# zachtong/RAFT-DVC

Hardware: AMD Instinct MI355X
Metric: corr build+lookup voxel-queries/s (128^3 pair, 1/4 encoder) (higher is better)
Workload: dtype bf16; 1 GPU; corr build + 12 lookups, 32^3 x 128 fmaps (128^3 input, 1/4 encoder), L=4, r=4, materialised, bf16 build / fp32 lookup; global_batch=1, query_voxels=32768, levels=4, radius=4, parallelism=single GPU, step_replay=hip graph after the collective

## Files before the change

### include/dvccorr.h

```cpp
#ifndef DVCCORR_H
#define DVCCORR_H

#include <stddef.h>
#include <stdint.h>

#ifdef __cplusplus
extern "C" {
#endif

#define DVC_MAX_LEVELS 8
#define DVC_ABI_VERSION 3
#define DVC_CORR_GUARD_BYTES 256

typedef enum {
    DVC_OK = 0,
    DVC_ERR_INVALID = 1,
    DVC_ERR_UNSUPPORTED = 2,
    DVC_ERR_LAUNCH = 3,
    DVC_ERR_RUNTIME = 4
} dvc_status;

typedef enum { DVC_F32 = 0, DVC_BF16 = 1, DVC_F16 = 2 } dvc_dtype;

#define DVC_BRICKED 0x100

typedef enum { DVC_FIXED = 0, DVC_LEGACY = 1 } dvc_convention;

typedef struct {
    int32_t num_levels;
    int32_t channels;
    int32_t c_pad;
    int32_t H[DVC_MAX_LEVELS];
    int32_t W[DVC_MAX_LEVELS];
    int32_t D[DVC_MAX_LEVELS];
    int32_t Dp[DVC_MAX_LEVELS];
    int32_t zero_level[DVC_MAX_LEVELS];
    int64_t offset[DVC_MAX_LEVELS];
    int64_t level_elems[DVC_MAX_LEVELS];
    int64_t row_elems;
    int64_t row_stride;
} dvc_layout;

int dvc_layout_init(int H, int W, int D, int num_levels, int C, dvc_layout *out);

int dvc_bricked_levels(const dvc_layout *lay);

size_t dvc_pack_workspace_bytes(int B, int C, int H, int W, int D, int num_levels);

int dvc_pack_queries(const float *fmap1, void *packed, int B, int C, int64_t Nq, int dtype, void *stream);

int dvc_pack_targets(const float *fmap2, void *packed, float *workspace, int B, int C, int H, int W, int D,
                     int num_levels, int dtype, void *stream);

int dvc_pack_targets_gathered(const float *gathered, int world, void *packed, int B, int C, int H, int W, int D,
                              int num_levels, int dtype, void *stream);

int dvc_corr_build(const void *packed_q, const void *packed_t, void *corr, int B, int64_t Nq, int C, int H, int W,
                   int D, int num_levels, int in_dtype, int store_dtype, int64_t col_begin, int64_t col_end,
                   void *stream);

int dvc_corr_pool(void *corr, int B, int64_t Nq, int H, int W, int D, int num_levels, int src_level,
                  int store_dtype, void *stream);

int dvc_corr_lookup(const void *corr, const float *coords, float *out, int B, int64_t Nq, int H, int W, int D,
                    int num_levels, int radius, int convention, int store_dtype, void *stream);

size_t dvc_lookup_fused_workspace_bytes(int B, int64_t Nq, int num_levels, int radius);
int dvc_corr_lookup_fused(const void *packed_q, const void *packed_t, const float *coords, float *out,
                          void *workspace, int B, int64_t Nq, int C, int H, int W, int D, int num_levels,
                          int radius, int convention, int dtype, void *stream);

size_t dvc_corr_backward_workspace_bytes(int B, int64_t Nq, int C, int H, int W, int D, int num_levels, int radius);
size_t dvc_corr_backward_workspace_bytes_dtype(int B, int64_t Nq, int C, int H, int W, int D, int num_levels,
                                               int radius, int dtype);
int dvc_corr_backward(const void *packed_q, const void *packed_t, const float *coords, const float *grad_out,
                      float *grad_fmap1, float *grad_fmap2, void *workspace, int B, int64_t Nq, int C, int H, int W,
                      int D, int num_levels, int radius, int convention, int dtype, void *stream);
int dvc_corr_backward_mfma(int B, int64_t Nq, int C, int H, int W, int D, int num_levels, int radius, int convention,
// ... 136 lines not shown
```

### raft-dvc_amd/csrc/capi.hip

```cpp
#include <math.h>
#include <stdarg.h>
#include <stdio.h>
#include <stdlib.h>
#include <string.h>

#include "common.h"
#include "lookup_common.h"

#include <type_traits>

namespace dvc {
__global__ void k_pool_fmap(const float *, float *, long long, int, int, int, int, int, int);
template <typename T>
__global__ void k_pack_rows(const float *, T *, int, int, long long, long long, int, int, long long, long long);
template <typename T, int CG> __global__ void k_pack_pyramid(const float *, T *, PyrGeo);
template <typename T> __global__ void k_pack_queries(const float *, T *, int, int, long long);
template <int NCH, bool STORE_F32, int ABL>
__global__ void k_build_bf16(const bf16_t *, const bf16_t *, bf16_t *, long long, int, long long, long long, long long,
                             long long, int, float);
template <int NCH, typename E>
__global__ void k_build_bf16_2b(const E *, const E *, E *, long long, int, long long, long long,
                                long long, long long, int, float, int);
__global__ void k_build_f32(const float *, const float *, float *, long long, int, long long, long long, long long,
                            long long, int, float);
// ... 138 lines not shown
}

static int volume_check(const char *what, int B, int H, int W, int D, const char *indices = "indices") {
    if (B < 1 || H < 1 || W < 1 || D < 1) return fail(DVC_ERR_INVALID, "%s: B=%d volume (%d,%d,%d)", what, B, H, W, D);
    const long long vox = (long long)B * H * W * D;
    if (vox >= (1LL << 31)) return fail(DVC_ERR_UNSUPPORTED, "%s: %lld voxels exceed 32-bit %s", what, vox, indices);
    return DVC_OK;
}

static inline long long ceil_div(long long a, long long b) { return (a + b - 1) / b; }
static inline long long round_up(long long a, long long b) { return ceil_div(a, b) * b; }

static int fill_lookup_args(LookupArgs &A, const dvc_layout &lay, const void *corr, const float *coords, float *out,
                            int B, long long Nq, int radius, int convention) {
    A.corr = corr; A.coords = coords; A.out = out;
    A.Nq = Nq; A.q0 = 0; A.nq = Nq; A.row_stride = lay.row_stride; A.nqb = ceil_div(Nq, 64);
    A.B = B; A.Ltot = lay.num_levels; A.l0 = 0; A.nl = lay.num_levels;
    A.legacy = convention == DVC_LEGACY; A.r = radius;
    const int n = 2 * radius + 1;
    A.ach = n >= 3 ? 3 : n;
    A.nach = (int)ceil_div(n, A.ach);
    for (int l = 0; l < DVC_MAX_LEVELS; ++l) {
        A.H[l] = lay.H[l]; A.W[l] = lay.W[l]; A.D[l] = lay.D[l]; A.Dp[l] = lay.Dp[l];
        A.zero[l] = lay.zero_level[l]; A.off[l] = lay.offset[l];
        A.generic[l] = l < lay.num_levels && A.legacy && lay.W[l] != lay.D[l];
    }
    A.ablate = g_lookup_ablate;
    A.order = g_lookup_order;
    A.ldpol = g_lookup_ldpol;
    A.proj_w = nullptr; A.proj_b = nullptr; A.proj_out = nullptr;
    A.trace = (unsigned long long *)(((unsigned long long)(unsigned)g_trace_hi << 32) | (unsigned)g_trace_lo);
    A.split_levels = 0;
    A.brick = 0;
    return DVC_OK;
}


static int lookup_variant() {
    if (g_lookup_variant < 0) {
        const char *e = getenv("DVCCORR_LOOKUP_VARIANT");
        g_lookup_variant = e ? atoi(e) : 2;
    }
    return g_lookup_variant;
}

static bool tile_ok(const LookupArgs &A, size_t esz) {
    return A.r >= 1 && A.r <= 6 && (long long)64 * A.row_stride * (long long)esz < (1LL << 31) - 4096;
}

static constexpr long long kSplitTiles = 1024, kSplitRows = 512;
static Knob<int> g_split_ach{5};
static Knob<long long> g_split_tiles{kSplitTiles};
static Knob<int> g_lookup_waves{4};
static Knob<int> g_lookup_stpol{-1};

template <typename T, bool NT, int ACH>
static void launch_tile_r(const LookupArgs &A, dim3 blocks, unsigned threads, hipStream_t s) {
    switch (A.r) {
    case 1: k_lookup_tile<T, 1, NT, 0, false, ACH><<<blocks, threads, 0, s>>>(A); break;
    case 2: k_lookup_tile<T, 2, NT, 0, false, ACH><<<blocks, threads, 0, s>>>(A); break;
    case 3: k_lookup_tile<T, 3, NT, 0, false, ACH><<<blocks, threads, 0, s>>>(A); break;
    case 4: k_lookup_tile<T, 4, NT, 0, false, ACH><<<blocks, threads, 0, s>>>(A); break;
    case 5: k_lookup_tile<T, 5, NT, 0, false, ACH><<<blocks, threads, 0, s>>>(A); break;
    case 6: k_lookup_tile<T, 6, NT, 0, false, ACH><<<blocks, threads, 0, s>>>(A); break;
    default: break;
    }
}

template <typename T, bool NT>
static void launch_tile_nt(const LookupArgs &A0, hipStream_t s) {
    LookupArgs A = A0;
    const long long tiles = (long long)A.B * A.nqb;
    A.split_levels = tiles < g_split_tiles && A.nl > 1;
    const int n = 2 * A.r + 1;
    const int ach = g_split_ach;
    const bool split_rows = NT && A.split_levels && tiles * A.nl < kSplitRows && n > ach && ach > 0;
    const dim3 blocks((unsigned)tiles, A.split_levels ? (unsigned)A.nl : 1u,
                      split_rows ? (unsigned)((n + ach - 1) / ach) : 1u);
    const bool bal = NT && A.r == 4 && g_lookup_waves == 4 && (ach == 5 || !split_rows);
    const unsigned threads = 64u * (bal ? 4u : (unsigned)((2 * A.r + 3) / 3));
#if DVC_DIAG
    if constexpr (std::is_same<T, bf16_t>::value && NT) {
        if (A.r == 4 && A.ablate >= 1 && A.ablate <= 4) {
            const dim3 b1((unsigned)tiles, blocks.y);
            if (A.ablate == 4) k_lookup_tile<T, 4, NT, 4, false, 0><<<b1, 192, 0, s>>>(A);
            else if (A.ablate == 1) k_lookup_tile<T, 4, NT, 1, false, 0><<<b1, 192, 0, s>>>(A);
            else if (A.ablate == 2) k_lookup_tile<T, 4, NT, 2, false, 0><<<b1, 192, 0, s>>>(A);
            else k_lookup_tile<T, 4, NT, 3, false, 0><<<b1, 192, 0, s>>>(A);
            return;
        }
    }
#endif
    if constexpr (NT) {
        if (bal) {
#if DVC_DIAG
            if constexpr (std::is_same<T, bf16_t>::value) {
                if (A.trace) {
                    if (split_rows) k_lookup_tile<T, 4, true, 8, false, 5, 4><<<blocks, threads, 0, s>>>(A);
                    else k_lookup_tile<T, 4, true, 8, false, 0, 4><<<blocks, threads, 0, s>>>(A);
                    return;
                }
            }
#endif
            if (split_rows) {
                k_lookup_tile<T, 4, true, 0, false, 5, 4><<<blocks, threads, 0, s>>>(A);
                return;
            }
#if DVC_DIAG
            if constexpr (std::is_same<T, bf16_t>::value) {
                switch (g_lookup_stpol) {
// ... 95 lines not shown
#endif
    if (!strcmp(key, "lookup_variant")) {
        if (value < 0 || value > 2) return fail(DVC_ERR_INVALID, "set_tuning: lookup_variant %d", value);
        g_lookup_variant = value;
        return DVC_OK;
    }
    if (!strcmp(key, "lookup_stretch")) {
        if (value != 0 && value != 1) return fail(DVC_ERR_INVALID, "set_tuning: lookup_stretch %d (0 or 1)", value);
        g_lookup_stretch = value;
        return DVC_OK;
    }
    if (!strcmp(key, "lookup_nt")) {
        g_lookup_nt = value != 0;
        return DVC_OK;
    }
    if (!strcmp(key, "lookup_order")) {
        g_lookup_order = value != 0;
        return DVC_OK;
    }
    if (!strcmp(key, "lookup_ldpol")) {
        if (value < 0 || value > 3) return fail(DVC_ERR_INVALID, "set_tuning: lookup_ldpol %d", value);
        g_lookup_ldpol = value;
        return DVC_OK;
    }
    if (!strcmp(key, "lookup_waves")) {
        if (value != 0 && value != 4) return fail(DVC_ERR_INVALID, "set_tuning: lookup_waves %d (0 or 4)", value);
        g_lookup_waves = value;
        return DVC_OK;
    }
    if (!strcmp(key, "lookup_stpol")) {
        if (value != -1 && value != 0 && value != 16 && value != 17 && value != 18)
            return fail(DVC_ERR_INVALID, "set_tuning: lookup_stpol %d (-1, 0, 16, 17 or 18)", value);
        g_lookup_stpol = value;
        return DVC_OK;
    }
    if (!strcmp(key, "split_tiles")) {
        if (value < 0) return fail(DVC_ERR_INVALID, "set_tuning: split_tiles %d", value);
        g_split_tiles = value;
        return DVC_OK;
    }
    if (!strcmp(key, "split_ach")) {
        if (value != 0 && value != 2 && value != 3 && value != 5)
            return fail(DVC_ERR_INVALID, "set_tuning: split_ach %d (0, 2, 3 or 5)", value);
        g_split_ach = value;
        return DVC_OK;
    }
    if (!strcmp(key, "brick_min_dp")) {
        if (value != 16 && value != 32) return fail(DVC_ERR_INVALID, "set_tuning: brick_min_dp %d (16 or 32)", value);
        g_brick_min_dp = value;
        return DVC_OK;
    }
    if (!strcmp(key, "build_stpol")) {
        g_build_stpol = value != 0;
        return DVC_OK;
    }
    if (!strcmp(key, "pack_cg")) {
        if (value != 0 && value != 8 && value != 16 && value != 32) return fail(DVC_ERR_INVALID, "set_tuning: pack_cg %d", value);
        g_pack_cg = value;
        return DVC_OK;
    }
    if (!strcmp(key, "pack_variant")) {
        if (value < 0 || value > 1) return fail(DVC_ERR_INVALID, "set_tuning: pack_variant %d", value);
        g_pack_variant = value;
        return DVC_OK;
    }
    if (!strcmp(key, "build_f32_variant")) {
// ... 432 lines not shown
            return fail(DVC_ERR_UNSUPPORTED, "lookup: a DVC_BRICKED pyramid needs the tile kernel (radius 1..6, "
                                             "no legacy W != D bricked level, lookup_variant 2)");
    }
    const long long items = (long long)A.nl * A.nach * B * A.nqb;
    const unsigned blocks = (unsigned)ceil_div(items, 4);
    hipStream_t s = (hipStream_t)stream;
    if (store_dtype == DVC_BF16) launch_lookup<bf16_t>(A, blocks, s);
    else if (store_dtype == DVC_F16) launch_lookup<f16_t>(A, blocks, s);
    else launch_lookup<float>(A, blocks, s);
    if ((rc = check_launch("corr_lookup"))) return rc;
    if (radius >= 1 && radius <= 6) {
        for (int l = 0; l < lay.num_levels; ++l) {
            if (!A.generic[l] || A.zero[l]) continue;
            LookupArgs G = A;
            G.l0 = l; G.nl = 1;
            bool staged = false;
            if (store_dtype == DVC_BF16) staged = launch_stretch<bf16_t>(G, lay, l, s);
            else if (store_dtype == DVC_F16) staged = launch_stretch<f16_t>(G, lay, l, s);
            else staged = launch_stretch<float>(G, lay, l, s);
            if (staged) {
                if ((rc = check_launch("corr_lookup_stretch"))) return rc;
                continue;
            }
            const unsigned gb = (unsigned)ceil_div((long long)G.nach * B * G.nqb, 4);
            if (store_dtype == DVC_BF16) k_lookup_generic<bf16_t><<<gb, 256, 0, s>>>(G);
            else if (store_dtype == DVC_F16) k_lookup_generic<f16_t><<<gb, 256, 0, s>>>(G);
            else k_lookup_generic<float><<<gb, 256, 0, s>>>(G);
            if ((rc = check_launch("corr_lookup_generic"))) return rc;
        }
    }
    return DVC_OK;
}

size_t dvc_proj_packed_bytes(int num_levels, int radius) {
    if (num_levels < 1 || num_levels > DVC_MAX_LEVELS || radius < 1 || radius > DVC_PROJ_MAX_RADIUS) return 0;
    const int n = 2 * radius + 1;
    return (size_t)num_levels * n * ((n + 2) / 3) * DVC_PROJ_COUT * 32 * sizeof(bf16_t);
}

int dvc_proj_pack(const float *weight, void *packed, int cout, int num_levels, int radius, int convention,
                  void *stream) {
    if (!weight || !packed) return fail(DVC_ERR_INVALID, "proj_pack: null pointer");
    if (cout != DVC_PROJ_COUT) return fail(DVC_ERR_UNSUPPORTED, "proj_pack: %d output channels (convc1 has %d)", cout,
                                           DVC_PROJ_COUT);
    if (num_levels < 1 || num_levels > DVC_MAX_LEVELS)
        return fail(DVC_ERR_INVALID, "proj_pack: num_levels=%d outside [1, %d]", num_levels, DVC_MAX_LEVELS);
    if (radius < 1 || radius > DVC_PROJ_MAX_RADIUS)
        return fail(DVC_ERR_UNSUPPORTED, "proj_pack: radius %d outside [1, %d]", radius, DVC_PROJ_MAX_RADIUS);
    if (convention != DVC_FIXED && convention != DVC_LEGACY)
        return fail(DVC_ERR_INVALID, "proj_pack: bad convention %d", convention);
    const long long total = (long long)(dvc_proj_packed_bytes(num_levels, radius) / sizeof(bf16_t));
    k_proj_pack<<<(unsigned)ceil_div(total, 256), 256, 0, (hipStream_t)stream>>>(
        weight, (bf16_t *)packed, num_levels, radius, convention == DVC_LEGACY, total, 0);
    return check_launch("proj_pack");
}

int dvc_proj_pack_exact(const float *weight, void *packed, int cout, int num_levels, int radius, int convention,
                        void *stream) {
    if (!weight || !packed) return fail(DVC_ERR_INVALID, "proj_pack_exact: null pointer");
    if (cout != DVC_PROJ_COUT)
        return fail(DVC_ERR_UNSUPPORTED, "proj_pack_exact: %d output channels (convc1 has %d)", cout, DVC_PROJ_COUT);
    if (num_levels < 1 || num_levels > DVC_MAX_LEVELS)
        return fail(DVC_ERR_INVALID, "proj_pack_exact: num_levels=%d outside [1, %d]", num_levels, DVC_MAX_LEVELS);
    if (radius < 1 || radius > DVC_PROJ_MAX_RADIUS)
        return fail(DVC_ERR_UNSUPPORTED, "proj_pack_exact: radius %d outside [1, %d]", radius, DVC_PROJ_MAX_RADIUS);
    if (convention != DVC_FIXED && convention != DVC_LEGACY)
// ... 631 lines not shown
```

### raft-dvc_amd/csrc/common.h

```cpp
#pragma once

#include <hip/hip_runtime.h>
#include <stdint.h>

#include <algorithm>
#include <atomic>

#include "dvccorr.h"

#ifndef DVC_DIAG
#define DVC_DIAG 0
#endif
#ifndef DVC_PROJ_XLP
#define DVC_PROJ_XLP 0
#endif

typedef __bf16 bf16x2 __attribute__((ext_vector_type(2)));
typedef __bf16 bf16x8 __attribute__((ext_vector_type(8)));
typedef _Float16 f16x2 __attribute__((ext_vector_type(2)));
typedef _Float16 f16x8 __attribute__((ext_vector_type(8)));
typedef float f32x2 __attribute__((ext_vector_type(2)));
typedef float f32x4 __attribute__((ext_vector_type(4)));
typedef float f32x8 __attribute__((ext_vector_type(8)));
typedef float f32x16 __attribute__((ext_vector_type(16)));
// ... 31 lines not shown
}

__device__ __forceinline__ float bf16_bits_to_f32(unsigned int h) { return __uint_as_float(h << 16); }

__device__ __forceinline__ bf16_t f32_to_bf16(float f) { return __builtin_bit_cast(bf16_t, (__bf16)f); }

template <typename T> __device__ __forceinline__ unsigned pack2_16(float a, float b);
template <> __device__ __forceinline__ unsigned pack2_16<bf16_t>(float a, float b) {
    return (unsigned)f32_to_bf16(a) | ((unsigned)f32_to_bf16(b) << 16);
}
template <> __device__ __forceinline__ unsigned pack2_16<f16_t>(float a, float b) {
    return (unsigned)__builtin_bit_cast(unsigned short, (f16_t)a) |
           ((unsigned)__builtin_bit_cast(unsigned short, (f16_t)b) << 16);
}
template <typename T> __device__ __forceinline__ float bits16_to_f32(unsigned h);
template <> __device__ __forceinline__ float bits16_to_f32<bf16_t>(unsigned h) { return __uint_as_float(h << 16); }
template <> __device__ __forceinline__ float bits16_to_f32<f16_t>(unsigned h) {
    return (float)__builtin_bit_cast(f16_t, (unsigned short)(h & 0xffffu));
}

struct LookupArgs {
    const void *corr;
    const float *coords;
    float *out;
    long long Nq, q0, nq, nqb, row_stride;
    int B, Ltot, l0, nl, legacy, nach, ach, r;
    int H[DVC_MAX_LEVELS], W[DVC_MAX_LEVELS], D[DVC_MAX_LEVELS], Dp[DVC_MAX_LEVELS], zero[DVC_MAX_LEVELS];
    int generic[DVC_MAX_LEVELS];
    int ablate;
    int order;
    int ldpol;
    int split_levels;
    int brick;
    long long off[DVC_MAX_LEVELS];
    const void *proj_w;
    const float *proj_b;
    float *proj_out;
    unsigned long long *trace;
};

template <typename T> struct StoreT;
template <> struct StoreT<float> {
    static __device__ __forceinline__ float load(const float *p) { return *p; }
    static __device__ __forceinline__ void store(float *p, float v) { *p = v; }
};
template <> struct StoreT<bf16_t> {
    static __device__ __forceinline__ float load(const bf16_t *p) { return bf16_bits_to_f32(*p); }
    static __device__ __forceinline__ void store(bf16_t *p, float v) { *p = f32_to_bf16(v); }
};
template <> struct StoreT<f16_t> {
    static __device__ __forceinline__ float load(const f16_t *p) { return (float)*p; }
    static __device__ __forceinline__ void store(f16_t *p, float v) { *p = (f16_t)v; }
};

__device__ __forceinline__ float norm_coord(float x, float snm1) {
#pragma clang fp contract(off)
    float t = 2.0f * x;
    float u = t / snm1;
    return u - 1.0f;
}
__device__ __forceinline__ float unnorm_coord(float g, float sum1) {
#pragma clang fp contract(off)
    float t = g + 1.0f;
    float u = t / 2.0f;
    return u * sum1;
}
// ... 52 lines not shown
```

### raft-dvc_amd/csrc/lookup_common.h

```cpp
#pragma once

#include "common.h"

namespace dvc {

struct Item {
    int l, ac, b;
    long long qi;
};

__device__ __forceinline__ bool decode_item(const LookupArgs &A, Item &it) {
    const long long item = (long long)blockIdx.x * 4 + __builtin_amdgcn_readfirstlane((int)(threadIdx.x >> 6));
    const long long bq = (long long)A.B * A.nqb;
    const long long per_l = (long long)A.nach * bq;
    if (item >= per_l * A.nl) return false;
    const int li = (int)(item / per_l);
    long long rem = item - (long long)li * per_l;
    it.l = A.l0 + li;
    it.ac = (int)(rem / bq);
    rem -= (long long)it.ac * bq;
    it.b = (int)(rem / A.nqb);
    it.qi = (rem - (long long)it.b * A.nqb) * 64 + (threadIdx.x & 63);
    return true;
}
// ... 8 lines not shown

struct WinAxes {
    float ph, pu, pv;
    float kh, ku, kv;
    float hs, un, uu, vn, vu;
    bool dead;
};

__device__ __forceinline__ void window_axes(float py, float px, float pz, int Hl, int Wl, int Dl, int legacy,
                                            WinAxes &ax) {
    ax.ph = py;
    ax.pu = legacy ? pz : px;
    ax.pv = legacy ? px : pz;
    ax.dead = !(fabsf(ax.ph) < 1e6f) || !(fabsf(ax.pu) < 1e6f) || !(fabsf(ax.pv) < 1e6f);
    if (ax.dead) { ax.ph = -1e5f; ax.pu = -1e5f; ax.pv = -1e5f; }
    ax.hs = (float)(Hl - 1);
    ax.un = legacy ? (float)(Dl - 1) : (float)(Wl - 1);
    ax.uu = (float)(Wl - 1);
    ax.vn = legacy ? (float)(Wl - 1) : (float)(Dl - 1);
    ax.vu = (float)(Dl - 1);
    ax.kh = floorf(ax.ph);
    ax.ku = floorf(ax.pu);
    ax.kv = floorf(ax.pv);
}

__device__ __forceinline__ void axis_weights(float p, float kp, int d, float sn, float su, float &w0, float &w1) {
#pragma clang fp contract(off)
    const float x = roundtrip(p + (float)d, sn, su);
    const float k = kp + (float)d;
    w1 = x - k;
    w0 = (k + 1.0f) - x;
}

constexpr int kStretchSE = 3;
struct StretchGeo {
    int WX, DX, RB, LS, NYB, WXF;
    long long boxe;
};

}
```

### raft-dvc_amd/csrc/lookup_tile.h

```cpp
#pragma once

#include "common.h"
#include "lookup_common.h"

#include <type_traits>

namespace dvc {

#ifndef DVC_TILE_CB16
#define DVC_TILE_CB16 16
#endif
#ifndef DVC_TILE_PD16
#define DVC_TILE_PD16 2
#endif
template <typename T, int R, int NWV = 0> struct TileCfg {
    static constexpr int n = 2 * R + 1;
    static constexpr int NW = 2 * R + 2;
    static constexpr int ES = (int)sizeof(T);
    static constexpr int CB = ES == 4 ? 8 : (R <= 4 ? DVC_TILE_CB16 : 16);
    static constexpr int CE = CB / ES;
    static constexpr int ZWMAX = (NW + CE - 1 + CE - 1) / CE * CE;
    static constexpr int NWAVES = NWV > 0 ? NWV : (n + 2) / 3;
    static constexpr int COLS = NWV > 0 ? (n + NWV - 1) / NWV : 3;
    static constexpr int THREADS = 64 * NWAVES;
// ... 43 lines not shown
}

template <int NW>
__device__ __forceinline__ void lds_run(const unsigned char *base, int addr, const f16_t *, float (&v)[NW]) {
    constexpr int K = NW / 2;
    const unsigned *p = reinterpret_cast<const unsigned *>(base + (addr & ~3));
    unsigned d[K + 1];
#pragma unroll
    for (int i = 0; i <= K; ++i) d[i] = p[i];
    const unsigned sh = (unsigned)(addr & 2);
#pragma unroll
    for (int i = 0; i < K; ++i) {
        const unsigned w = __builtin_amdgcn_alignbyte(d[i + 1], d[i], sh);
        v[2 * i] = bits16_to_f32<f16_t>(w);
        v[2 * i + 1] = bits16_to_f32<f16_t>(w >> 16);
    }
}

template <int NW>
__device__ __forceinline__ void lds_run(const unsigned char *base, int addr, const float *, float (&v)[NW]) {
    const float *p = reinterpret_cast<const float *>(base + addr);
#pragma unroll
    for (int i = 0; i < NW; ++i) v[i] = p[i];
}

template <int n> struct ZRun {
    f32x2 p[n / 2];
    float t;
};

struct ProjCfg {
    static constexpr int COUT = 96, OT = COUT / 16, KW = 32;
};

#ifndef DVC_PROJ_ABL
#define DVC_PROJ_ABL 0
#endif
template <typename T, int R, bool NT, int ABL, int PROJ, int ACH, int NWV = 0, int SPOL = -1, bool XLP = false>
__global__ __launch_bounds__(64 * (TileCfg<T, R, NWV>::NWAVES + (PROJ ? 1 : 0)), PROJ == 2 ? 1 : 2) void k_lookup_tile(
    LookupArgs A) {
    using C = TileCfg<T, R, NWV>;
    static_assert(!PROJ || NWV == 0, "the convc1 weight packing assumes the 3-column waves");
    constexpr bool BAL = NWV > 0;
    constexpr int FLO = BAL ? C::n / C::NWAVES : 0, REM = BAL ? C::n % C::NWAVES : 0;
    constexpr int n = C::n, NW = C::NW, ES = C::ES, CE = C::CE, NP = n / 2;
    constexpr long long n3 = (long long)n * n * n;
    constexpr int NU_LAST = n - C::COLS * (C::NWAVES - 1);
    constexpr int XROW = C::NWAVES * ProjCfg::KW * 2 + 16;
    static_assert(!PROJ || C::COLS * n <= ProjCfg::KW, "PROJ: one wave's row values must fit a 32-k slice");
    __shared__ __attribute__((aligned(16))) unsigned char smem[C::LDS];
    __shared__ int tab[5][64];
    __shared__ __attribute__((aligned(16))) unsigned char xs[PROJ ? PROJ * 64 * XROW : 16];
    static_assert(PROJ != 2 || std::is_same<T, float>::value, "the split convc1 is the fp32 pyramid's");

    const int tid = threadIdx.x;
    const int lane = tid & 63;
    const int wave = __builtin_amdgcn_readfirstlane(tid >> 6);
    const int b = blockIdx.x / (int)A.nqb;
    const long long qb = blockIdx.x - (long long)b * A.nqb;
    const long long qt = qb * 64;
    const int nvalid = (int)min(64LL, A.nq - qt);
    const long long q = A.q0 + qt + lane;
    const bool active = lane < nvalid;
    const long long Nq = A.Nq;
    const bool rev = A.order && !A.split_levels && (blockIdx.x & 1);

    if constexpr (PROJ) {
        if (wave == C::NWAVES) {
            constexpr int OT = ProjCfg::OT, NWP = C::NWAVES;
            const int m16 = lane & 15, h4 = lane >> 4;
            f32x4 acc[OT][4];
#pragma unroll
            for (int ot = 0; ot < OT; ++ot)
#pragma unroll
                for (int j = 0; j < 4; ++j) acc[ot][j] = f32x4{0.f, 0.f, 0.f, 0.f};
            const f16x8 *wp = reinterpret_cast<const f16x8 *>(A.proj_w) + lane;
            const long long wlo = PROJ == 2 ? (long long)A.Ltot * n * NWP * OT * 64 : 0;
            const bool xlp_c = XLP && !A.split_levels;
            bool started_c = false;
            for (int li = 0; li < A.nl; ++li) {
                const int l = A.l0 + (rev ? A.nl - 1 - li : li);
                if (A.zero[l] || A.generic[l]) continue;
                if (!(xlp_c && started_c)) {
// ... 74 lines not shown
                for (int i = 0; i < 4; ++i) {
                    const int o = 16 * ot + 4 * h4 + i;
                    const float bo = A.proj_b[o];
#pragma unroll
                    for (int j = 0; j < 4; ++j) {
                        const int qq = 16 * j + m16;
                        const float v = acc[ot][j][i] + bo;
                        if (qq < nvalid) ob[(long long)o * Nq + qq] = v < 0.f ? 0.f : v;
                    }
                }
            return;
        }
    }

    const long long wg = ((long long)blockIdx.z * gridDim.y + blockIdx.y) * gridDim.x + blockIdx.x;
    int trace_level = 1;
    int trace_li = 0;
    auto stamp = [&](int k) {
        if constexpr ((ABL & 16) != 0) {
            if (tid == 0 && k < 16)
                __builtin_amdgcn_raw_buffer_store_b64(
                    __builtin_bit_cast(u32x2, (unsigned long long)__builtin_amdgcn_s_memrealtime()),
                    __builtin_amdgcn_make_buffer_rsrc(A.trace, (short)0, 0x7fffffff, 0x00020000),
                    (int)((wg * 64 + (k == 15 ? 3 : trace_li) * 16 + k) * 8), 0, 0);
        } else if constexpr ((ABL & 8) != 0) {
            if (tid == 0 && (trace_level || k == 15) && k < 16)
                __builtin_amdgcn_raw_buffer_store_b64(
                    __builtin_bit_cast(u32x2, (unsigned long long)__builtin_amdgcn_s_memrealtime()),
                    __builtin_amdgcn_make_buffer_rsrc(A.trace, (short)0, 0x7fffffff, 0x00020000),
                    (int)((wg * 16 + k) * 8), 0, 0);
        }
    };
    stamp(0);
    float cy = 0.f, cx = 0.f, cz = 0.f;
    if (active) load_coords(A.coords, b, Nq, q, cy, cx, cz);
    for (int i = tid * 16; i < C::LDS; i += C::THREADS * 16) *reinterpret_cast<u32x4 *>(smem + i) = u32x4{0, 0, 0, 0};

    const T *tile_rows = reinterpret_cast<const T *>(A.corr) + ((long long)b * Nq + A.q0 + qt) * A.row_stride;
    const unsigned long long trp = (unsigned long long)tile_rows;
    const unsigned trlo = __builtin_amdgcn_readfirstlane((unsigned)trp);
    const unsigned trhi = __builtin_amdgcn_readfirstlane((unsigned)(trp >> 32));
    const int nrec = __builtin_amdgcn_readfirstlane((int)((long long)nvalid * A.row_stride * ES));
    const __amdgpu_buffer_rsrc_t rs_in = __builtin_amdgcn_make_buffer_rsrc(
        (void *)(((unsigned long long)trhi << 32) | trlo), (short)0, nrec, 0x00020000);
    const int q4 = active ? (int)(q * 4) : 0x7ffffff0;
    const int chstep_u = A.legacy ? 1 : n;
    const int chstep_v = A.legacy ? n : 1;
    const int u0 = BAL ? wave * FLO + min(wave, REM) : wave * C::COLS;

    auto out_rsrc = [&](float *obase, int a, int u) {
        return __builtin_amdgcn_make_buffer_rsrc(obase + ((long long)a * n * n + (long long)u * chstep_u) * Nq,
                                                 (short)0, (int)(n * n * Nq * 4), 0x00020000);
    };
    auto store = [&](__amdgpu_buffer_rsrc_t rs, int v, float val) {
        if constexpr ((ABL & 1) != 0) asm volatile("" ::"v"(val));
        else __builtin_amdgcn_raw_buffer_store_b32(__float_as_uint(val), rs, q4, (int)(v * chstep_v * Nq * 4),
                                                   SPOL >= 0 ? SPOL : (NT ? 2 : 0));
    };

    static_assert(!PROJ || ACH == 0, "the convc1 consumer accumulates every row of the tile");
    using Chunk = typename std::conditional<C::CB == 16, u32x4, u32x2>::type;
    constexpr int PD = PROJ ? 2 : C::PD;
    const bool xlp = XLP && ACH == 0 && PD == 2 && !A.split_levels;
    Chunk st_x[PD][C::MAXCH];
    int voff[C::MAXCH];
    unsigned pk[C::MAXCH];
// ... 298 lines not shown
                u32x4 *dst = reinterpret_cast<u32x4 *>(xs + lane * XROW + wave * (ProjCfg::KW * 2));
#pragma unroll
                for (int j = 0; j < ProjCfg::KW / 8; ++j)
                    dst[j] = u32x4{xw[4 * j], xw[4 * j + 1], xw[4 * j + 2], xw[4 * j + 3]};
                if constexpr (PROJ == 2) {
                    u32x4 *dl = reinterpret_cast<u32x4 *>(xs + 64 * XROW + lane * XROW + wave * (ProjCfg::KW * 2));
#pragma unroll
                    for (int j = 0; j < ProjCfg::KW / 8; ++j)
                        dl[j] = u32x4{xwl[4 * j], xwl[4 * j + 1], xwl[4 * j + 2], xwl[4 * j + 3]};
                }
            }
            if (ia + 2 < NPL) {
                write_plane(ia & 1, a + 2, st[(ia + 2) % PD]);
                if (PD > 2 && ia + 2 + PD < NPL) load_plane(a + 2 + PD, g.plane_bytes, st[(ia + 2) % PD]);
            }
            if constexpr (XLP && PD == 2 && NA >= 3) {
                if (ia == NA - 3 && lnx >= 0 && wave == 0) {
                    const LevelGeo gn = geo(lnx);
                    WinAxes axn;
                    int ihn, iun, ivn, csn, zan;
                    window(lnx, gn, axn, ihn, iun, ivn, csn, zan);
                    write_tab(gn, ihn, csn, zan, ivn, iun);
                }
                if (ia == NA - 1 && lnx >= 0) {
                    write_plane(0, 0, st[0]);
                    load_plane(2, gx.plane_bytes, st[0]);
                }
            }
            __syncthreads();
            stamp(6 + ia);
        }
    };

    const int li0 = A.split_levels ? (int)blockIdx.y : 0;
    const int li1 = A.split_levels ? li0 + 1 : A.nl;
    constexpr int NCH_A = ACH > 0 ? (n + ACH - 1) / ACH : 1;
    constexpr int NA_FULL = ACH > 0 ? ACH : n;
    constexpr int NA_TAIL = ACH > 0 ? n - ACH * (NCH_A - 1) : n;
    const int a0 = ACH > 0 ? (int)blockIdx.z * ACH : 0;
    auto rows = [&](int l, auto nu_c, bool pre, int lnx) {
        if (NA_TAIL == NA_FULL || a0 + NA_FULL <= n) level(l, nu_c, std::integral_constant<int, NA_FULL>{}, a0, pre, lnx);
        else level(l, nu_c, std::integral_constant<int, NA_TAIL>{}, a0, pre, lnx);
    };
    auto walk_level = [&](int li) { return A.l0 + (rev ? A.nl - 1 - li : li); };
    auto runs = [&](int l) { return !A.zero[l] && !A.generic[l]; };
    bool started = false;
    for (int li = li0; li < li1; ++li) {
        const int l = walk_level(li);
        if (A.generic[l] && !A.zero[l]) continue;
        int lnx = -1;
        if (xlp && runs(l))
            for (int lj = li + 1; lj < li1 && lnx < 0; ++lj)
                if (runs(walk_level(lj))) lnx = walk_level(lj);
        const bool pre = xlp && started && runs(l);
        if constexpr (BAL) {
            if (REM > 0 && wave < REM) rows(l, std::integral_constant<int, FLO + 1>{}, pre, lnx);
            else rows(l, std::integral_constant<int, FLO>{}, pre, lnx);
        } else if (NU_LAST == C::COLS || wave < C::NWAVES - 1) {
            rows(l, std::integral_constant<int, C::COLS>{}, pre, lnx);
        } else {
            rows(l, std::integral_constant<int, NU_LAST>{}, pre, lnx);
        }
        started |= runs(l);
        trace_level = 0;
        ++trace_li;
    }
    stamp(15);
// ... 4 lines not shown
```

### raft-dvc_amd/dvccorr/_lib.py

```python
from __future__ import annotations

import ctypes
import os

_HERE = os.path.dirname(os.path.abspath(__file__))
LIB_PATH = os.environ.get("DVCCORR_LIB") or os.path.join(_HERE, "libdvccorr.so")

DVC_OK, DVC_ERR_INVALID, DVC_ERR_UNSUPPORTED, DVC_ERR_LAUNCH, DVC_ERR_RUNTIME = range(5)
DVC_F32, DVC_BF16, DVC_F16 = 0, 1, 2
DVC_BRICKED = 0x100
DVC_FIXED, DVC_LEGACY = 0, 1
MAX_LEVELS = 8

EXPORTED = (
    "dvc_layout_init", "dvc_pack_workspace_bytes", "dvc_pack_queries", "dvc_pack_targets", "dvc_pack_targets_gathered",
    "dvc_corr_build",
    "dvc_corr_pool", "dvc_corr_lookup", "dvc_lookup_fused_workspace_bytes", "dvc_corr_lookup_fused",
    "dvc_sample3d", "dvc_set_tuning", "dvc_last_error", "dvc_version", "dvc_abi_version",
    "dvc_corr_backward_workspace_bytes", "dvc_corr_backward_workspace_bytes_dtype", "dvc_corr_backward",
    "dvc_proj_packed_bytes", "dvc_proj_pack", "dvc_proj_pack_exact",
    "dvc_corr_lookup_proj", "dvc_lookup_fused_proj_workspace_bytes", "dvc_corr_lookup_fused_proj",
    "dvc_coords_grid", "dvc_upflow", "dvc_flow_step", "dvc_bricked_levels", "dvc_corr_backward_mfma", "dvc_corr_backward_gout64",
    "dvc_gru_packed_bytes", "dvc_gru_pack", "dvc_sep_gru_pass",
    "dvc_conv3_packed_bytes", "dvc_conv3_pack", "dvc_conv3",
    "dvc_conv7_flow_packed_bytes", "dvc_conv7_flow_pack", "dvc_conv7_flow",
    "dvc_conv3_pack_dgrad", "dvc_conv3_grad_prep", "dvc_conv3_wgrad_workspace_bytes", "dvc_conv3_wgrad",
    "dvc_sep_gru_pass_save", "dvc_gru_dgrad_packed_bytes", "dvc_gru_pack_dgrad", "dvc_gru_grad_prep",
    "dvc_sep_gru_dgrad", "dvc_gru_wgrad_workspace_bytes", "dvc_gru_wgrad",
    "dvc_conv7_wgrad_workspace_bytes", "dvc_conv7_wgrad",
    "dvc_enc_stem_packed_bytes", "dvc_enc_stem_pack", "dvc_enc_stem",
    "dvc_enc_conv_packed_bytes", "dvc_enc_conv_pack", "dvc_enc_conv",
    "dvc_enc_partials_bytes", "dvc_enc_stats", "dvc_enc_residual",
)
PROJ_COUT = 96
PROJ_MAX_RADIUS = 4
GRU_HIDDEN = 96
GRU_MAX_INPUT = 160
GRU_SEG = 8
CONV3_TH, CONV3_TW, CONV3_TD = 4, 4, 16
CONV3_MAX_CIN = 128
CONV3_MAX_COUT = 128
CONV3_WGRAD_KH, CONV3_WGRAD_KW, CONV3_WGRAD_KD = 4, 4, 16
CONV3_WGRAD_TARGET = 512
CONV3_PREP_CHUNK = 4096
GRU_WGRAD_LINES, GRU_WGRAD_POS, GRU_WGRAD_TARGET = 32, 4, 512
CONV7_TH, CONV7_TW, CONV7_TD = 4, 4, 16
CONV7_COUT = 64
CONV7_WGRAD_KH, CONV7_WGRAD_KW, CONV7_WGRAD_KD = 4, 4, 16
CONV7_WGRAD_TILES = 5
CONV7_WGRAD_TARGET = 256
ENC_TH, ENC_TW, ENC_TD = 4, 4, 16
ENC_STEM_COUT = 32
ENC_MAX_CIN, ENC_MAX_COUT = 128, 160
ENC_IDENTITY, ENC_RELU, ENC_NORM_RELU = 0, 1, 2
ENC_SC_PLAIN, ENC_SC_NORM, ENC_SC_NORM_RELU = 0, 1, 2
# ... 9 lines not shown
        ("W", ctypes.c_int32 * MAX_LEVELS),
        ("D", ctypes.c_int32 * MAX_LEVELS),
        ("Dp", ctypes.c_int32 * MAX_LEVELS),
        ("zero_level", ctypes.c_int32 * MAX_LEVELS),
        ("offset", ctypes.c_int64 * MAX_LEVELS),
        ("level_elems", ctypes.c_int64 * MAX_LEVELS),
        ("row_elems", ctypes.c_int64),
        ("row_stride", ctypes.c_int64),
    ]

    def levels(self):
        return [(self.H[l], self.W[l], self.D[l]) for l in range(self.num_levels)]


class DvcError(RuntimeError):
    """A HIP launch/runtime failure reported by libdvccorr."""


_lib = None


def lib() -> ctypes.CDLL:
    global _lib
    if _lib is not None:
        return _lib
    if not os.path.exists(LIB_PATH):
        raise ImportError(f"{LIB_PATH} is missing: build it with `make -C raft-dvc_amd/csrc` "
                          "(hipcc --offload-arch=gfx950); there is no CPU fallback")
    L = ctypes.CDLL(LIB_PATH)
    i32, i64, vp, sz = ctypes.c_int, ctypes.c_int64, ctypes.c_void_p, ctypes.c_size_t
    sig = {
        "dvc_layout_init": (i32, [i32, i32, i32, i32, i32, ctypes.POINTER(Layout)]),
        "dvc_bricked_levels": (i32, [ctypes.POINTER(Layout)]),
        "dvc_pack_workspace_bytes": (sz, [i32, i32, i32, i32, i32, i32]),
        "dvc_pack_queries": (i32, [vp, vp, i32, i32, i64, i32, vp]),
        "dvc_pack_targets": (i32, [vp, vp, vp, i32, i32, i32, i32, i32, i32, i32, vp]),
        "dvc_pack_targets_gathered": (i32, [vp, i32, vp, i32, i32, i32, i32, i32, i32, i32, vp]),
        "dvc_corr_build": (i32, [vp, vp, vp, i32, i64, i32, i32, i32, i32, i32, i32, i32, i64, i64, vp]),
        "dvc_corr_pool": (i32, [vp, i32, i64, i32, i32, i32, i32, i32, i32, vp]),
        "dvc_corr_lookup": (i32, [vp, vp, vp, i32, i64, i32, i32, i32, i32, i32, i32, i32, vp]),
        "dvc_lookup_fused_workspace_bytes": (sz, [i32, i64, i32, i32]),
        "dvc_corr_lookup_fused": (i32, [vp, vp, vp, vp, vp, i32, i64, i32, i32, i32, i32, i32, i32, i32, i32, vp]),
        "dvc_sample3d": (i32, [vp, vp, vp, i32, i32, i32, i32, i32, i64, i32, vp]),
        "dvc_corr_backward_workspace_bytes": (sz, [i32, i64, i32, i32, i32, i32, i32, i32]),
        "dvc_corr_backward_workspace_bytes_dtype": (sz, [i32, i64, i32, i32, i32, i32, i32, i32, i32]),
        "dvc_corr_backward": (i32, [vp, vp, vp, vp, vp, vp, vp, i32, i64, i32, i32, i32, i32, i32, i32, i32, i32,
                                    vp]),
        "dvc_corr_backward_mfma": (i32, [i32, i64, i32, i32, i32, i32, i32, i32, i32, i32]),
        "dvc_corr_backward_gout64": (i32, [i64, i32]),
        "dvc_proj_packed_bytes": (sz, [i32, i32]),
        "dvc_proj_pack": (i32, [vp, vp, i32, i32, i32, i32, vp]),
        "dvc_proj_pack_exact": (i32, [vp, vp, i32, i32, i32, i32, vp]),
        "dvc_corr_lookup_proj": (i32, [vp, vp, vp, vp, vp, i32, i64, i32, i32, i32, i32, i32, i32, i32, vp]),
        "dvc_lookup_fused_proj_workspace_bytes": (sz, [i32, i64]),
        "dvc_corr_lookup_fused_proj": (i32, [vp, vp, vp, vp, vp, vp, vp, i32, i64, i32, i32, i32, i32, i32, i32, i32,
                                             i32, vp]),
        "dvc_coords_grid": (i32, [vp, i32, i32, i32, i32, vp]),
        "dvc_upflow": (i32, [vp, vp, i32, i32, i32, i32, i32, i32, i32, i32, vp]),
        "dvc_flow_step": (i32, [vp, vp, vp, vp, i32, i32, i32, i32, i32, i32, i32, vp]),
        "dvc_gru_packed_bytes": (sz, [i32, i32, i32]),
        "dvc_gru_pack": (i32, [vp, vp, vp, vp, vp, vp, vp, i32, i32, i32, vp]),
        "dvc_sep_gru_pass": (i32, [vp, vp, vp, vp, i32, i32, i32, i32, i32, i32, i32, i32, vp]),
        "dvc_conv3_packed_bytes": (sz, [i32, i32, i32]),
        "dvc_conv3_pack": (i32, [vp, vp, vp, i32, i32, i32, vp]),
        "dvc_conv3": (i32, [vp, i32, vp, i32, vp, vp, i32, i32, i32, i32, i32, i32, i32, i32, i32, vp]),
        "dvc_conv3_pack_dgrad": (i32, [vp, vp, i32, i32, i32, vp]),
# ... 28 lines not shown
    }
    for name, (res, args) in sig.items():
        fn = getattr(L, name)
        fn.restype, fn.argtypes = res, args
    _lib = L
    return L


def check(rc: int, what: str = "") -> None:
    if rc == DVC_OK:
        return
    msg = lib().dvc_last_error().decode(errors="replace")
    if what:
        msg = f"{what}: {msg}"
    if rc == DVC_ERR_INVALID:
        raise ValueError(msg)
    if rc == DVC_ERR_UNSUPPORTED:
        raise NotImplementedError(msg)
    raise DvcError(msg)


def set_tuning(key: str, value: int) -> None:
    check(lib().dvc_set_tuning(key.encode(), int(value)), "set_tuning")


def layout(H: int, W: int, D: int, num_levels: int, C: int = 1) -> Layout:
    lay = Layout()
    rc = lib().dvc_layout_init(H, W, D, num_levels, C, ctypes.byref(lay))
    if rc != DVC_OK:
        raise RuntimeError(lib().dvc_last_error().decode(errors="replace"))
    return lay


def bricked_levels(lay: Layout) -> int:
    return int(lib().dvc_bricked_levels(ctypes.byref(lay)))
```

Baseline: 187.6 million voxel-queries/s.

## Add coarse-level lookup path staging whole small levels in LDS and merging them

```diff
diff --git a/include/dvccorr.h b/include/dvccorr.h
--- a/include/dvccorr.h
+++ b/include/dvccorr.h
@@ -44,6 +44,9 @@
 int dvc_layout_init(int H, int W, int D, int num_levels, int C, dvc_layout *out);
 
 int dvc_bricked_levels(const dvc_layout *lay);
+
+int dvc_lookup_coarse_levels(int B, int64_t Nq, int H, int W, int D, int num_levels, int radius, int convention,
+                             int store_dtype);
 
 size_t dvc_pack_workspace_bytes(int B, int C, int H, int W, int D, int num_levels);
 
diff --git a/raft-dvc_amd/csrc/capi.hip b/raft-dvc_amd/csrc/capi.hip
--- a/raft-dvc_amd/csrc/capi.hip
+++ b/raft-dvc_amd/csrc/capi.hip
@@ -194,6 +194,7 @@
     A.trace = (unsigned long long *)(((unsigned long long)(unsigned)g_trace_hi << 32) | (unsigned)g_trace_lo);
     A.split_levels = 0;
     A.brick = 0;
+    A.ncoarse = 0; A.coarse_merge = 0; A.coarse_first = 0;
     return DVC_OK;
 }
 
@@ -215,6 +216,19 @@
 static Knob<long long> g_split_tiles{kSplitTiles};
 static Knob<int> g_lookup_waves{4};
 static Knob<int> g_lookup_stpol{-1};
+
+static Knob<int> g_lookup_coarse{1};
+
+static int coarse_count(const LookupArgs &A, int esz) {
+    int k = 0;
+    if (!g_lookup_coarse || !A.split_levels || A.ablate) return 0;
+    for (int l = A.l0 + A.nl - 1; l >= A.l0; --l) {
+        if (A.zero[l] || A.generic[l] || ((A.brick >> l) & 1) || !coarse_level_ok(A.H[l], A.W[l], A.Dp[l], esz, A.r))
+            break;
+        ++k;
+    }
+    return k;
+}
 
 template <typename T, bool NT, int ACH>
 static void launch_tile_r(const LookupArgs &A, dim3 blocks, unsigned threads, hipStream_t s) {
@@ -237,7 +251,12 @@
     const int n = 2 * A.r + 1;
     const int ach = g_split_ach;
     const bool split_rows = NT && A.split_levels && tiles * A.nl < kSplitRows && n > ach && ach > 0;
-    const dim3 blocks((unsigned)tiles, A.split_levels ? (unsigned)A.nl : 1u,
+    const int cmode = g_lookup_coarse;
+    A.ncoarse = coarse_count(A, (int)sizeof(T));
+    A.coarse_merge = cmode == 1 || cmode == 3;
+    A.coarse_first = cmode == 1 || cmode == 4;
+    const int units = A.nl - A.ncoarse + (A.ncoarse > 0 && A.coarse_merge ? 1 : A.ncoarse);
+    const dim3 blocks((unsigned)tiles, A.split_levels ? (unsigned)units : 1u,
                       split_rows ? (unsigned)((n + ach - 1) / ach) : 1u);
     const bool bal = NT && A.r == 4 && g_lookup_waves == 4 && (ach == 5 || !split_rows);
     const unsigned threads = 64u * (bal ? 4u : (unsigned)((2 * A.r + 3) / 3));
@@ -399,6 +418,11 @@
         if (value != -1 && value != 0 && value != 16 && value != 17 && value != 18)
             return fail(DVC_ERR_INVALID, "set_tuning: lookup_stpol %d (-1, 0, 16, 17 or 18)", value);
         g_lookup_stpol = value;
+        return DVC_OK;
+    }
+    if (!strcmp(key, "lookup_coarse")) {
+        if (value < 0 || value > 4) return fail(DVC_ERR_INVALID, "set_tuning: lookup_coarse %d (0..4)", value);
+        g_lookup_coarse = value;
         return DVC_OK;
     }
     if (!strcmp(key, "split_tiles")) {
@@ -897,6 +921,22 @@
     return DVC_OK;
 }
 
+int dvc_lookup_coarse_levels(int B, int64_t Nq, int H, int W, int D, int num_levels, int radius, int convention,
+                             int store_dtype) {
+    dvc_layout lay;
+    if (dvc_layout_init(H, W, D, num_levels, 1, &lay) || B < 1 || Nq < 1 || radius < 0 || radius > 16) return -1;
+    const bool bricked = (store_dtype & DVC_BRICKED) != 0;
+    store_dtype &= ~DVC_BRICKED;
+    if (store_dtype != DVC_BF16 && store_dtype != DVC_F32 && store_dtype != DVC_F16) return -1;
+    LookupArgs A;
+    fill_lookup_args(A, lay, nullptr, nullptr, nullptr, B, Nq, radius, convention);
+    const int esz = store_dtype == DVC_F32 ? 4 : 2;
+    if (bricked) A.brick = dvc_bricked_levels(&lay);
+    if (lookup_variant() != 2 || !tile_ok(A, (size_t)esz)) return 0;
+    A.split_levels = (long long)A.B * A.nqb < g_split_tiles && A.nl > 1;
+    return coarse_count(A, esz);
+}
+
 size_t dvc_proj_packed_bytes(int num_levels, int radius) {
     if (num_levels < 1 || num_levels > DVC_MAX_LEVELS || radius < 1 || radius > DVC_PROJ_MAX_RADIUS) return 0;
     const int n = 2 * radius + 1;
diff --git a/raft-dvc_amd/csrc/common.h b/raft-dvc_amd/csrc/common.h
--- a/raft-dvc_amd/csrc/common.h
+++ b/raft-dvc_amd/csrc/common.h
@@ -87,6 +87,9 @@
     int ldpol;
     int split_levels;
     int brick;
+    int ncoarse;
+    int coarse_merge;
+    int coarse_first;
     long long off[DVC_MAX_LEVELS];
     const void *proj_w;
     const float *proj_b;
diff --git a/raft-dvc_amd/csrc/lookup_coarse.h b/raft-dvc_amd/csrc/lookup_coarse.h
--- /dev/null
+++ b/raft-dvc_amd/csrc/lookup_coarse.h
@@ -0,0 +1,189 @@
+#pragma once
+
+namespace dvc {
+
+template <typename T, int R, bool NT, int ABL, int SPOL, int NU, int THREADS, typename Stamp, typename Done>
+__device__ __forceinline__ void coarse_unit(const LookupArgs &A, unsigned char *smem, int lc0, int lc1, int u0, int a0,
+                                            int a1, int b, long long qt, int nvalid, Stamp &&stamp, Done &&done) {
+    constexpr int n = 2 * R + 1, NW = 2 * R + 2, ES = (int)sizeof(T), NP = n / 2;
+    constexpr long long n3 = (long long)n * n * n;
+    constexpr int GUARD = kCoarseGuard, PAD = kCoarsePad;
+    constexpr int KB = 16;
+    constexpr int OOB = 0x7fff0000;
+    static_assert(GUARD >= NW * ES + 4, "a clamped run may start NW elements before / end NW + 2 past the image");
+    const int tid = threadIdx.x;
+    const int lane = tid & 63;
+    const long long Nq = A.Nq;
+    const long long q = A.q0 + qt + lane;
+    const bool active = lane < nvalid;
+
+    const T *tile_rows = reinterpret_cast<const T *>(A.corr) + ((long long)b * Nq + A.q0 + qt) * A.row_stride;
+    const unsigned long long trp = (unsigned long long)tile_rows;
+    const unsigned trlo = __builtin_amdgcn_readfirstlane((unsigned)trp);
+    const unsigned trhi = __builtin_amdgcn_readfirstlane((unsigned)(trp >> 32));
+    const int nrec = __builtin_amdgcn_readfirstlane((int)((long long)nvalid * A.row_stride * ES));
+    const __amdgpu_buffer_rsrc_t rs_in = __builtin_amdgcn_make_buffer_rsrc(
+        (void *)(((unsigned long long)trhi << 32) | trlo), (short)0, nrec, 0x00020000);
+    const int rs_b = (int)A.row_stride * ES;
+    const int q4 = active ? (int)(q * 4) : 0x7ffffff0;
+    const int chstep_u = A.legacy ? 1 : n;
+    const int chstep_v = A.legacy ? n : 1;
+    auto out_rsrc = [&](float *obase, int a, int u) {
+        return __builtin_amdgcn_make_buffer_rsrc(obase + ((long long)a * n * n + (long long)u * chstep_u) * Nq,
+                                                 (short)0, (int)(n * n * Nq * 4), 0x00020000);
+    };
+    auto store = [&](__amdgpu_buffer_rsrc_t rs, int v, float val) {
+        if constexpr ((ABL & 1) != 0) asm volatile("" ::"v"(val));
+        else __builtin_amdgcn_raw_buffer_store_b32(__float_as_uint(val), rs, q4, (int)(v * chstep_v * Nq * 4),
+                                                   SPOL >= 0 ? SPOL : (NT ? 2 : 0));
+    };
+
+    float cy = 0.f, cx = 0.f, cz = 0.f;
+    if (active) load_coords(A.coords, b, Nq, q, cy, cx, cz);
+
+    for (int l = lc0; l < lc1; ++l) {
+        const int Hl = A.H[l], Wl = A.W[l], Dl = A.D[l], Dpl = A.Dp[l];
+        const int img_b = Hl * Wl * Dpl * ES;
+        const int SQ = img_b + PAD;
+        const int cpq = img_b >> 4;
+        const int nch = 64 * cpq;
+        const int lev_b = (int)A.off[l] * ES;
+        const float inv_cpq = 1.0f / (float)cpq;
+        if (l > lc0) __syncthreads();
+
+        u32x4 st[KB];
+        int lo[KB];
+        auto issue = [&](int base) {
+#pragma unroll
+            for (int k = 0; k < KB; ++k) {
+                const int idx = base + tid + k * THREADS;
+                int j = (int)((float)idx * inv_cpq);
+                int c = idx - j * cpq;
+                if (c < 0) { --j; c += cpq; }
+                else if (c >= cpq) { ++j; c -= cpq; }
+                const bool ok = idx < nch;
+                lo[k] = ok ? GUARD + j * SQ + c * 16 : -1;
+                st[k] = __builtin_bit_cast(
+                    u32x4, __builtin_amdgcn_raw_buffer_load_b128(rs_in, ok ? j * rs_b + lev_b + c * 16 : OOB, 0, 0));
+            }
+        };
+        auto commit = [&]() {
+#pragma unroll
+            for (int k = 0; k < KB; ++k)
+                if (lo[k] >= 0) {
+                    *reinterpret_cast<u32x2 *>(smem + lo[k]) = u32x2{st[k][0], st[k][1]};
+                    *reinterpret_cast<u32x2 *>(smem + lo[k] + 8) = u32x2{st[k][2], st[k][3]};
+                }
+        };
+        issue(0);
+        if (tid < 64) *reinterpret_cast<u32x2 *>(smem + GUARD + tid * SQ + img_b) = u32x2{0, 0};
+        if (tid < GUARD / 8) {
+            *reinterpret_cast<u32x2 *>(smem + tid * 8) = u32x2{0, 0};
+            *reinterpret_cast<u32x2 *>(smem + GUARD + 64 * SQ + tid * 8) = u32x2{0, 0};
+        }
+
+        float *obase = A.out + ((long long)b * A.Ltot + l) * n3 * Nq;
+        const float sc = (float)(1 << l);
+        WinAxes ax;
+        window_axes(cy / sc, cx / sc, cz / sc, Hl, Wl, Dl, A.legacy, ax);
+        const int ih = (int)ax.kh - R, iu = (int)ax.ku - R, iv = (int)ax.kv - R;
+        float wv0[n], wv1[n];
+#pragma unroll
+        for (int t = 0; t < n; ++t) {
+            axis_weights(ax.pv, ax.kv, t - R, ax.vn, ax.vu, wv0[t], wv1[t]);
+            wv0[t] = (unsigned)(iv + t) < (unsigned)Dl ? wv0[t] : 0.0f;
+            wv1[t] = (unsigned)(iv + t + 1) < (unsigned)Dl ? wv1[t] : 0.0f;
+        }
+        f32x2 w0p[NP], w1p[NP];
+#pragma unroll
+        for (int i = 0; i < NP; ++i) {
+            w0p[i] = f32x2{wv0[2 * i], wv0[2 * i + 1]};
+            w1p[i] = f32x2{wv1[2 * i], wv1[2 * i + 1]};
+        }
+        float wx0[NU], wx1[NU];
+#pragma unroll
+        for (int uu = 0; uu < NU; ++uu) {
+            const int u = u0 + uu;
+            axis_weights(ax.pu, ax.ku, u - R, ax.un, ax.uu, wx0[uu], wx1[uu]);
+            wx0[uu] = (unsigned)(iu + u) < (unsigned)Wl ? wx0[uu] : 0.0f;
+            wx1[uu] = (unsigned)(iu + u + 1) < (unsigned)Wl ? wx1[uu] : 0.0f;
+        }
+        const int rz = min(max(iv, -NW), Dpl);
+        const int plane_b = Wl * Dpl * ES;
+        int coff[NU + 1];
+#pragma unroll
+        for (int k = 0; k <= NU; ++k) {
+            const int xc = min(max(iu + u0 + k, 0), Wl - 1);
+            coff[k] = GUARD + lane * SQ + (xc * Dpl + rz) * ES;
+        }
+        constexpr bool BF = std::is_same<T, bf16_t>::value;
+        unsigned sel_e = 0, sel_o = 0;
+        if constexpr (BF) bf16_run_selectors((rz & 1) != 0, sel_e, sel_o);
+        auto lerp_col = [&](int y, int k, ZRun<n> &z) {
+            const int addr = coff[k] + min(max(y, 0), Hl - 1) * plane_b;
+            float r[NW];
+            if constexpr (BF) lds_run_perm<NW>(smem, addr, sel_e, sel_o, r);
+            else lds_run<NW>(smem, addr, (const T *)nullptr, r);
+#pragma unroll
+            for (int i = 0; i < NP; ++i)
+                z.p[i] = __builtin_elementwise_fma(f32x2{r[2 * i + 1], r[2 * i + 2]}, w1p[i],
+                                                   f32x2{r[2 * i], r[2 * i + 1]} * w0p[i]);
+            z.t = __builtin_fmaf(r[n], wv1[n - 1], r[n - 1] * wv0[n - 1]);
+        };
+        stamp(1);
+
+        commit();
+        for (int base = THREADS * KB; base < nch; base += THREADS * KB) {
+            issue(base);
+            commit();
+        }
+        stamp(3);
+        __syncthreads();
+        stamp(4);
+
+        ZRun<n> zp[NU + 1];
+#pragma unroll
+        for (int k = 0; k <= NU; ++k) lerp_col(ih + a0, k, zp[k]);
+        stamp(5);
+        for (int a = a0; a < a1; ++a) {
+            float wy0, wy1;
+            axis_weights(ax.ph, ax.kh, a - R, ax.hs, ax.hs, wy0, wy1);
+            wy0 = (unsigned)(ih + a) < (unsigned)Hl ? wy0 : 0.0f;
+            wy1 = (unsigned)(ih + a + 1) < (unsigned)Hl ? wy1 : 0.0f;
+            ZRun<n> zprev;
+#pragma unroll
+            for (int k = 0; k <= NU; ++k) {
+                ZRun<n> zcur;
+                lerp_col(ih + a + 1, k, zcur);
+                if (k >= 1) {
+                    const int uu = k - 1;
+                    const float p00 = wx0[uu] * wy0, p10 = wx1[uu] * wy0;
+                    const float p01 = wx0[uu] * wy1, p11 = wx1[uu] * wy1;
+                    const f32x2 P00 = {p00, p00}, P10 = {p10, p10}, P01 = {p01, p01}, P11 = {p11, p11};
+                    const __amdgpu_buffer_rsrc_t rs = out_rsrc(obase, a, u0 + uu);
+#pragma unroll
+                    for (int i = 0; i < NP; ++i) {
+                        f32x2 acc = P00 * zp[uu].p[i];
+                        acc = __builtin_elementwise_fma(P10, zp[uu + 1].p[i], acc);
+                        acc = __builtin_elementwise_fma(P01, zprev.p[i], acc);
+                        acc = __builtin_elementwise_fma(P11, zcur.p[i], acc);
+                        store(rs, 2 * i, acc[0]);
+                        store(rs, 2 * i + 1, acc[1]);
+                    }
+                    float acc = p00 * zp[uu].t;
+                    acc = __builtin_fmaf(p10, zp[uu + 1].t, acc);
+                    acc = __builtin_fmaf(p01, zprev.t, acc);
+                    acc = __builtin_fmaf(p11, zcur.t, acc);
+                    store(rs, n - 1, acc);
+                    zp[uu] = zprev;
+                }
+                zprev = zcur;
+                if (k == NU) zp[k] = zcur;
+            }
+            if (6 + a - a0 < 15) stamp(6 + a - a0);
+        }
+        done();
+    }
+}
+
+}
diff --git a/raft-dvc_amd/csrc/lookup_common.h b/raft-dvc_amd/csrc/lookup_common.h
--- a/raft-dvc_amd/csrc/lookup_common.h
+++ b/raft-dvc_amd/csrc/lookup_common.h
@@ -64,6 +64,14 @@
     w0 = (k + 1.0f) - x;
 }
 
+constexpr int kCoarsePad = 8, kCoarseGuard = 64;
+constexpr bool coarse_instance(int esz, int r) { return esz == 2 && r >= 1 && r <= 4; }
+constexpr int coarse_row_bytes(int r) { return r <= 2 ? 256 : 1024; }
+constexpr int coarse_lds(int r) { return 2 * kCoarseGuard + 64 * (coarse_row_bytes(r) + kCoarsePad); }
+inline bool coarse_level_ok(int Hl, int Wl, int Dpl, int esz, int r) {
+    return coarse_instance(esz, r) && (long long)Hl * Wl * Dpl * esz <= coarse_row_bytes(r);
+}
+
 constexpr int kStretchSE = 3;
 struct StretchGeo {
     int WX, DX, RB, LS, NYB, WXF;
diff --git a/raft-dvc_amd/csrc/lookup_tile.h b/raft-dvc_amd/csrc/lookup_tile.h
--- a/raft-dvc_amd/csrc/lookup_tile.h
+++ b/raft-dvc_amd/csrc/lookup_tile.h
@@ -99,6 +99,12 @@
 struct ProjCfg {
     static constexpr int COUT = 96, OT = COUT / 16, KW = 32;
 };
+}
+
+#include "lookup_coarse.h"
+
+namespace dvc {
+
 
 #ifndef DVC_PROJ_ABL
 #define DVC_PROJ_ABL 0
@@ -115,7 +121,9 @@
     constexpr int NU_LAST = n - C::COLS * (C::NWAVES - 1);
     constexpr int XROW = C::NWAVES * ProjCfg::KW * 2 + 16;
     static_assert(!PROJ || C::COLS * n <= ProjCfg::KW, "PROJ: one wave's row values must fit a 32-k slice");
-    __shared__ __attribute__((aligned(16))) unsigned char smem[C::LDS];
+    constexpr bool COARSE = !PROJ && coarse_instance(C::ES, R);
+    constexpr int SMEM = (COARSE && coarse_lds(R) > C::LDS) ? coarse_lds(R) : C::LDS;
+    __shared__ __attribute__((aligned(16))) unsigned char smem[SMEM];
     __shared__ int tab[5][64];
     __shared__ __attribute__((aligned(16))) unsigned char xs[PROJ ? PROJ * 64 * XROW : 16];
     static_assert(PROJ != 2 || std::is_same<T, float>::value, "the split convc1 is the fp32 pyramid's");
@@ -256,6 +264,37 @@
         }
     };
     stamp(0);
+    int unit = (int)blockIdx.y;
+    if constexpr (COARSE) {
+        if (A.ncoarse > 0) {
+            const int nfine = A.nl - A.ncoarse, ncu = (int)gridDim.y - nfine;
+            if (A.coarse_first) unit = unit < ncu ? nfine + unit : unit - ncu;
+            if (unit >= nfine) {
+                const int lc0 = A.l0 + (A.coarse_merge ? nfine : unit);
+                const int lc1 = A.coarse_merge ? A.l0 + A.nl : lc0 + 1;
+                const int ca0 = ACH > 0 ? (int)blockIdx.z * ACH : 0;
+                const int ca1 = ACH > 0 ? min(ca0 + ACH, C::n) : C::n;
+                const int cu0 = BAL ? wave * FLO + min(wave, REM) : wave * C::COLS;
+                auto coarse = [&](auto nu_c) {
+                    coarse_unit<T, R, NT, ABL, SPOL, decltype(nu_c)::value, C::THREADS>(
+                        A, smem, lc0, lc1, cu0, ca0, ca1, b, qt, nvalid, stamp, [&]() {
+                            trace_level = 0;
+                            ++trace_li;
+                        });
+                };
+                if constexpr (BAL) {
+                    if (REM > 0 && wave < REM) coarse(std::integral_constant<int, FLO + 1>{});
+                    else coarse(std::integral_constant<int, FLO>{});
+                } else if (NU_LAST == C::COLS || wave < C::NWAVES - 1) {
+                    coarse(std::integral_constant<int, C::COLS>{});
+                } else {
+                    coarse(std::integral_constant<int, NU_LAST>{});
+                }
+                stamp(15);
+                return;
+            }
+        }
+    }
     float cy = 0.f, cx = 0.f, cz = 0.f;
     if (active) load_coords(A.coords, b, Nq, q, cy, cx, cz);
     for (int i = tid * 16; i < C::LDS; i += C::THREADS * 16) *reinterpret_cast<u32x4 *>(smem + i) = u32x4{0, 0, 0, 0};
@@ -620,7 +659,7 @@
         }
     };
 
-    const int li0 = A.split_levels ? (int)blockIdx.y : 0;
+    const int li0 = A.split_levels ? unit : 0;
     const int li1 = A.split_levels ? li0 + 1 : A.nl;
     constexpr int NCH_A = ACH > 0 ? (n + ACH - 1) / ACH : 1;
     constexpr int NA_FULL = ACH > 0 ? ACH : n;
diff --git a/raft-dvc_amd/dvccorr/_lib.py b/raft-dvc_amd/dvccorr/_lib.py
--- a/raft-dvc_amd/dvccorr/_lib.py
+++ b/raft-dvc_amd/dvccorr/_lib.py
@@ -20,7 +20,7 @@
     "dvc_corr_backward_workspace_bytes", "dvc_corr_backward_workspace_bytes_dtype", "dvc_corr_backward",
     "dvc_proj_packed_bytes", "dvc_proj_pack", "dvc_proj_pack_exact",
     "dvc_corr_lookup_proj", "dvc_lookup_fused_proj_workspace_bytes", "dvc_corr_lookup_fused_proj",
-    "dvc_coords_grid", "dvc_upflow", "dvc_flow_step", "dvc_bricked_levels", "dvc_corr_backward_mfma", "dvc_corr_backward_gout64",
+    "dvc_coords_grid", "dvc_upflow", "dvc_flow_step", "dvc_bricked_levels", "dvc_lookup_coarse_levels", "dvc_corr_backward_mfma", "dvc_corr_backward_gout64",
     "dvc_gru_packed_bytes", "dvc_gru_pack", "dvc_sep_gru_pass",
     "dvc_conv3_packed_bytes", "dvc_conv3_pack", "dvc_conv3",
     "dvc_conv7_flow_packed_bytes", "dvc_conv7_flow_pack", "dvc_conv7_flow",
@@ -96,6 +96,7 @@
     sig = {
         "dvc_layout_init": (i32, [i32, i32, i32, i32, i32, ctypes.POINTER(Layout)]),
         "dvc_bricked_levels": (i32, [ctypes.POINTER(Layout)]),
+        "dvc_lookup_coarse_levels": (i32, [i32, ctypes.c_int64, i32, i32, i32, i32, i32, i32, i32]),
         "dvc_pack_workspace_bytes": (sz, [i32, i32, i32, i32, i32, i32]),
         "dvc_pack_queries": (i32, [vp, vp, i32, i32, i64, i32, vp]),
         "dvc_pack_targets": (i32, [vp, vp, vp, i32, i32, i32, i32, i32, i32, i32, vp]),
@@ -190,5 +191,10 @@
     return lay
 
 
+def lookup_coarse_levels(B: int, Nq: int, H: int, W: int, D: int, num_levels: int, radius: int, legacy: bool,
+                         store_dtype: int) -> int:
+    return int(lib().dvc_lookup_coarse_levels(B, Nq, H, W, D, num_levels, radius, 1 if legacy else 0, store_dtype))
+
+
 def bricked_levels(lay: Layout) -> int:
     return int(lib().dvc_bricked_levels(ctypes.byref(lay)))
```

Measured after the change: 202.7 million voxel-queries/s (median of 6 runs). 1.08x the previous value.
